# renjie-liang/HUAL

Measured on AMD Instinct MI355X. Metric: train clips/sec, higher is better.
Workload: dtype f32 (fp16x3 / bf16x3 split-operand MFMA, fp32 accumulate); 1 GPU; Charades-STA SeqPAN train step (fwd+bwd+clip+AdamWD, dropout 0.2), batch 64/GPU, T=128, vdim=1024, L=20, C=8, dim=128, 8 heads, 2 attention layers, random init; ONE batch resident in HBM, batch assembly (hual_assemble_batch) outside the timed region; global_batch=64, T=128, vdim=1024, L=20, parallelism=dp1, launch=hipGraph, video_dtype=f32

## Files before the change

hual_amd/csrc/dablock.h:

```cpp
#pragma once
#include "common.h"
#include "rowops.h"

namespace hual {

#define HUAL_LNPROJ_MAX 5
struct LnProjArgs {
  const float* x;
  const float* xa; int pre_site; float* x_out;
  uint8_t* pre_bits; uint8_t* y1_bits;
  const float* x2;
  const float* g1; const float* b1; float* y1;
  int drop_site1;
  const float* g2; const float* b2; float* y2;
  float* mean; float* rstd;
  int nproj;
  const float* wimg[HUAL_LNPROJ_MAX];
  const float* bias[HUAL_LNPROJ_MAX];
  float* out[HUAL_LNPROJ_MAX]; int ldo[HUAL_LNPROJ_MAX];
  int src[HUAL_LNPROJ_MAX];
  int accum[HUAL_LNPROJ_MAX];
  int act[HUAL_LNPROJ_MAX];
  int out_site[HUAL_LNPROJ_MAX];
  uint8_t* out_bits[HUAL_LNPROJ_MAX];
// ... 51 lines not shown
  const float* pre_x; const float* pre_mean; const float* pre_rstd; const float* pre_g; const float* pre_dy; const float* pre_add;
};
int ln_proj_bwd_rows(int R, int Nv = 0);
int ln_proj_bwd_blocks(int R, int Nv = 0);
int launch_ln_proj_bwd(const LnProjBwdArgs& a, const DropCfg& drop, hipStream_t s);

struct DaMidBwdArgs {
  const float* dz1;
  const float *gate, *val, *sg, *xg, *sv, *xv;
  const float* w[10];
  float *d_sc, *d_val, *d_ln1a, *d_g, *dz_sg, *dz_xg, *d_sv, *d_xv, *d_satt, *d_xatt;
  int R; int MT; int Nv;
};
int launch_da_mid_bwd(const DaMidBwdArgs& a, hipStream_t s);

}
```

hual_amd/csrc/dablock.hip:

```cpp
#include "dablock.h"
#include "tilecore.h"
#include "prof.h"

using namespace hual;

__device__ __forceinline__ float row16_max(float v) {
  v = fmaxf(v, dpp_xor_partner(v, 1));
  v = fmaxf(v, dpp_xor_partner(v, 2));
  v = fmaxf(v, dpp_xor_partner(v, 4));
  v = fmaxf(v, dpp_xor_partner(v, 8));
  return v;
}
__device__ __forceinline__ float4 sig4(float4 v) { return make_float4(sigmoidf_(v.x), sigmoidf_(v.y), sigmoidf_(v.z), sigmoidf_(v.w)); }

#include "lnproj_body.h"

template <int NT, bool PLAIN>
__global__ __launch_bounds__(CB_THREADS) void ln_proj_kernel(LnProjArgs a, DropCfg drop) {
  extern __shared__ __attribute__((aligned(16))) char lp_lds[];
  ln_proj_body<NT, false, PLAIN>(a, drop, lp_lds);
}
template <int NT>
__global__ __launch_bounds__(CB_THREADS) void ln_proj_pair_kernel(LnProjArgs a0, LnProjArgs a1, DropCfg drop) {
  extern __shared__ __attribute__((aligned(16))) char lp_lds[];
// ... 271 lines not shown
  }
}
template <int NT>
__global__ __launch_bounds__(CB_THREADS) void da_post_kernel(DaPostArgs a, DropCfg drop) {
  extern __shared__ __attribute__((aligned(16))) char dp_lds[];
  da_post_body<NT, false>(a, drop, nullptr, dp_lds);
}
template <int NT>
__global__ __launch_bounds__(CB_THREADS) void da_post_lnproj_kernel(DaPostArgs a, DropCfg drop, LnProjArgs lp) {
  extern __shared__ __attribute__((aligned(16))) char dp_lds[];
  da_post_body<NT, true>(a, drop, &lp, dp_lds);
}

#define LB_ROWS 48
#define LB_U (LB_ROWS / 16)
template <bool PRE, int NT, bool SIX = false>
__global__ __launch_bounds__(CB_THREADS) void ln_proj_bwd_kernel(LnProjBwdArgs a, DropCfg drop) {
  extern __shared__ __attribute__((aligned(16))) char lb_lds[];
  char* S0 = lb_lds;
  char* S1 = S0 + 2 * LB_ROWS * 256;
  char* Ps = S1 + 2 * LB_ROWS * 256;
  float* ainv0 = reinterpret_cast<float*>(Ps + 8 * 4 * 32 * 16);
  float* ainv1 = ainv0 + LB_ROWS;
  const int lane = threadIdx.x & 63, wave = threadIdx.x >> 6;
  const int l32 = threadIdx.x & 31, grp = threadIdx.x >> 5;
  const int col = 4 * l32;
  const int MT = a.MT, R = a.R;
  const int tile_ = xcd_tile_clip(blockIdx.x, R, a.Nv, MT);
  if (tile_ < 0) return;
  const int r0 = tile_ * MT;
  const int RE = min(R, r0 + MT);
  const int j = lane & 15, g = lane >> 4, ecol = 16 * wave + 4 * g;
  const DropRegs dr = drop_load(drop);

  TfW w[2];
  tf_load_w(w[0], a.wimg_t[0], wave, lane);
  float4 nv[LB_U], xv[LB_U], a1v[LB_U];
  float mu[LB_U], rsd[LB_U];
  constexpr bool pre = PRE;
  const float* add1p = pre ? (a.pre_add ? a.pre_add : a.x) : (a.add1 ? a.add1 : a.x);
  const float* a0p = pre ? a.pre_dy : a.A[0];
  const int lda0 = pre ? HUAL_D : a.lda[0];
  uint32_t nkb[LB_U];
  const int nsteps = SIX ? 6 : a.nsteps;
  auto has_bits = [&](int k) { return !SIX && a.a_bits[k] != nullptr; };
  auto to_second = [&](int k) { return SIX ? k >= 4 : a.dst[k] != 0; };
  const bool has_g2 = SIX || a.g2 != nullptr, has_add_dy1 = SIX || a.add_dy1 != nullptr, has_dy1_bits = !SIX && a.dy1_bits != nullptr;
  const uint8_t* kb0p = has_bits(0) ? a.a_bits[0] : reinterpret_cast<const uint8_t*>(a.x);
  float4 pxv[LB_U];
  float pmu[LB_U], prs[LB_U];
#pragma unroll
  for (int u = 0; u < LB_U; ++u) {
    const int row = min(r0 + grp + 16 * u, R - 1);
    nv[u] = ld4(a0p + (size_t)row * lda0 + col);
    nkb[u] = SIX ? 0u : kb0p[(size_t)row * 16 + (l32 >> 1)];
    xv[u] = ld4(a.x + (size_t)row * HUAL_D + col);
    a1v[u] = ld4(add1p + (size_t)row * HUAL_D + col);
    mu[u] = a.mean[row];
    rsd[u] = a.rstd[row];
    if (pre) { pxv[u] = ld4(a.pre_x + (size_t)row * HUAL_D + col); pmu[u] = a.pre_mean[row]; prs[u] = a.pre_rstd[row]; }
  }
  const float4 g1 = ld4(a.g1 + col);
  float4 sg2 = f4zero(), sb2 = f4zero();
  if (pre) {
    const float4 pg = ld4(a.pre_g + col);
#pragma unroll
    for (int u = 0; u < LB_U; ++u) {
      const int lr = grp + 16 * u;
      const bool ok = lr < MT && r0 + lr < RE;
      const float4 v = pxv[u], dy = nv[u];
      const float mean = pmu[u], rstd = prs[u];
      const float4 xh = make_float4((v.x - mean) * rstd, (v.y - mean) * rstd, (v.z - mean) * rstd, (v.w - mean) * rstd);
      if (ok) { sb2 = cb_add(sb2, dy); sg2 = cb_fma(dy, xh, sg2); }
      const float4 gv = cb_mul(dy, pg);
      const float m1 = fast_sum32(cb_hsum(gv)) * (1.0f / HUAL_D);
      const float m2 = fast_sum32(cb_hsum(cb_mul(gv, xh))) * (1.0f / HUAL_D);
      float4 dx = make_float4(rstd * (gv.x - m1 - xh.x * m2), rstd * (gv.y - m1 - xh.y * m2),
                              rstd * (gv.z - m1 - xh.z * m2), rstd * (gv.w - m1 - xh.w * m2));
      if (a.pre_add) dx = make_float4(__fadd_rn(dx.x, a1v[u].x), __fadd_rn(dx.y, a1v[u].y), __fadd_rn(dx.z, a1v[u].z), __fadd_rn(dx.w, a1v[u].w));
      nv[u] = dx;
      a1v[u] = dx;
    }
  }
  const float4 g2 = has_g2 ? ld4(a.g2 + col) : f4zero();
  float4 addt[NT];
  const float* addp = has_add_dy1 ? a.add_dy1 : a.x;
#pragma unroll
  for (int rt = 0; rt < NT; ++rt) addt[rt] = SIX ? f4zero() : ld4(addp + (uint32_t)min(r0 + 16 * rt + j, R - 1) * (uint32_t)HUAL_D + (uint32_t)ecol);
  auto fill = [&](int k) {
    char* S = (k & 1) ? S1 : S0;
    float* ai = (k & 1) ? ainv1 : ainv0;
#pragma unroll
    for (int u = 0; u < LB_U; ++u) {
      const int lr = grp + 16 * u, row = r0 + lr;
      if (lr >= MT) continue;
      const bool ok = row < RE;
      float4 v = ok ? nv[u] : f4zero();
      if (has_bits(k)) {
        if (dr.enabled) v = f4_select((nkb[u] >> (4 * (l32 & 1))) & 15u, make_float4(v.x * dr.scale, v.y * dr.scale, v.z * dr.scale, v.w * dr.scale));
        if (ok && a.a_save[k]) st4_nt(a.a_save[k] + (size_t)row * HUAL_D + col, v);
      }
      const float inv = cb_store_operand(S, S + LB_ROWS * 256, lr, l32, v);
      if (l32 == 0) ai[lr] = ok ? inv : 0.f;
// ... 1 lines not shown
  };
  HUAL_STAMP_K(4, 0);
  fill(0);
  HUAL_STAMP_K(4, 1);
  float4 acc0[NT], acc1[NT];
  bool first0 = true, first1 = true;
#pragma unroll
  for (int rt = 0; rt < NT; ++rt) { acc0[rt] = f4zero(); acc1[rt] = f4zero(); }
#pragma unroll
  for (int k = 0; k < HUAL_LNBWD_MAX; ++k) {
    if (k >= nsteps) break;
    const bool more = k + 1 < nsteps;
    if (SIX && k == 5) {
#pragma unroll
      for (int rt = 0; rt < NT; ++rt) addt[rt] = ld4(addp + (uint32_t)min(r0 + 16 * rt + j, R - 1) * (uint32_t)HUAL_D + (uint32_t)ecol);
    }
    if (more) {
      const uint8_t* nbp = has_bits(k + 1) ? a.a_bits[k + 1] : reinterpret_cast<const uint8_t*>(a.x);
      const float* nap = a.A[k + 1];
      const int nld = a.lda[k + 1];
#pragma unroll
      for (int u = 0; u < LB_U; ++u) {
        const size_t row = (size_t)min(r0 + grp + 16 * u, R - 1);
        nv[u] = ld4(nap + row * nld + col);
        nkb[u] = SIX ? 0u : nbp[row * 16 + (l32 >> 1)];
      }
      tf_load_w(w[(k + 1) & 1], a.wimg_t[k + 1], wave, lane);
    }
    cb_barrier();
    HUAL_STAMP_K(4, 2 + 3 * k);
// ... 28 lines not shown
    float4 v = acc0[rt];
    if (has_add_dy1) v = cb_add(v, addt[rt]);
    D0[lr * 32 + (ecol >> 2)] = v;
    if (has_g2) D1[lr * 32 + (ecol >> 2)] = acc1[rt];
  }
  uint32_t kb1[LB_U], kbz[LB_U];
  {
    const uint8_t* b1p = has_dy1_bits ? a.dy1_bits : reinterpret_cast<const uint8_t*>(a.x);
    const uint8_t* bzp = a.dz_bits ? a.dz_bits : reinterpret_cast<const uint8_t*>(a.x);
#pragma unroll
    for (int u = 0; u < LB_U; ++u) {
      const size_t row = (size_t)min(r0 + grp + 16 * u, R - 1);
      kb1[u] = SIX ? 0u : b1p[row * 16 + (l32 >> 1)];
      kbz[u] = bzp[row * 16 + (l32 >> 1)];
    }
  }
  cb_barrier();
  HUAL_STAMP_K(4, 21);
  float4 sg1 = f4zero(), sb1 = f4zero();
#pragma unroll
  for (int u = 0; u < LB_U; ++u) {
    const int lr = grp + 16 * u, row = r0 + lr;
    if (lr >= MT || row >= R) continue;
    const size_t off = (size_t)row * HUAL_D + col;
    const float4 v = xv[u];
    const float mean = mu[u], rstd = rsd[u];
    const float4 xh = make_float4((v.x - mean) * rstd, (v.y - mean) * rstd, (v.z - mean) * rstd, (v.w - mean) * rstd);
    float4 dy = D0[lr * 32 + l32];
    if (has_dy1_bits && dr.enabled) dy = f4_select((kb1[u] >> (4 * (l32 & 1))) & 15u, make_float4(dy.x * dr.scale, dy.y * dr.scale, dy.z * dr.scale, dy.w * dr.scale));
    sb1 = cb_add(sb1, dy);
    sg1 = cb_fma(dy, xh, sg1);
    float4 gv = cb_mul(dy, g1);
    if (has_g2) {
      const float4 dy2 = D1[lr * 32 + l32];
      sb2 = cb_add(sb2, dy2);
      sg2 = cb_fma(dy2, xh, sg2);
      gv = cb_fma(dy2, g2, gv);
    }
    const float m1 = fast_sum32(cb_hsum(gv)) * (1.0f / HUAL_D);
    const float m2 = fast_sum32(cb_hsum(cb_mul(gv, xh))) * (1.0f / HUAL_D);
    float4 dx = make_float4(rstd * (gv.x - m1 - xh.x * m2), rstd * (gv.y - m1 - xh.y * m2),
                            rstd * (gv.z - m1 - xh.z * m2), rstd * (gv.w - m1 - xh.w * m2));
    if (SIX || a.add1 || pre) dx = make_float4(__fadd_rn(dx.x, a1v[u].x), __fadd_rn(dx.y, a1v[u].y), __fadd_rn(dx.z, a1v[u].z), __fadd_rn(dx.w, a1v[u].w));
    st4(a.dx + off, dx);
    if (a.dz) {
      if (a.dz_bits && dr.enabled) dx = f4_select((kbz[u] >> (4 * (l32 & 1))) & 15u, make_float4(dx.x * dr.scale, dx.y * dr.scale, dx.z * dr.scale, dx.w * dr.scale));
      st4(a.dz + off, dx);
    }
  }
  HUAL_STAMP_K(4, 22);
  {
    auto xor32_sum = [&](float v) {
      const unsigned x = __builtin_bit_cast(unsigned, v);
      const auto r = __builtin_amdgcn_permlane32_swap(x, x, false, false);
      return v + __builtin_bit_cast(float, (lane & 32) ? r[0] : r[1]);
    };
    auto xor32_sum4 = [&](float4 v) { return make_float4(xor32_sum(v.x), xor32_sum(v.y), xor32_sum(v.z), xor32_sum(v.w)); };
    sg1 = xor32_sum4(sg1); sb1 = xor32_sum4(sb1); sg2 = xor32_sum4(sg2); sb2 = xor32_sum4(sb2);
    float4* pb = reinterpret_cast<float4*>(Ps);
    if (lane < 32) {
      float4* dst = pb + wave * 4 * 32 + l32;
      dst[0] = sg1; dst[32] = sb1; dst[64] = sg2; dst[96] = sb2;
    }
    cb_barrier();
    const float* pf = reinterpret_cast<const float*>(pb);
    const int e = threadIdx.x;
    float s = 0.f;
#pragma unroll
    for (int w = 0; w < 8; ++w) s += pf[w * 4 * HUAL_D + e];
    a.part[(size_t)tile_ * 4 * HUAL_D + e] = s;
  }
  HUAL_STAMP_K(4, 23);
}

template <int NT>
__global__ __launch_bounds__(CB_THREADS) void da_mid_bwd_kernel(DaMidBwdArgs a) {
  extern __shared__ __attribute__((aligned(16))) char dm_lds[];
  char* P0 = dm_lds;
  char* P1 = P0 + DP_SLOT;
  char* P2 = P1 + DP_SLOT;
  float* ainv0 = reinterpret_cast<float*>(P2 + DP_SLOT);
  float* ainv1 = ainv0 + DP_ROWS;
  float* ainv2 = ainv1 + DP_ROWS;
  float* smaxA = ainv2 + DP_ROWS;
  float* smaxB = smaxA + 8 * DP_ROWS;
  const int lane = threadIdx.x & 63, wave = threadIdx.x >> 6;
  const int l32 = threadIdx.x & 31, grp = threadIdx.x >> 5;
  const int col = 4 * l32;
  const int MT = a.MT, R = a.R;
  const int tile_ = xcd_tile_clip(blockIdx.x, R, a.Nv, MT);
  if (tile_ < 0) return;
  const int r0 = tile_ * MT;
  const int RE = min(R, r0 + MT);
  const int j = lane & 15, g = lane >> 4, ecol = 16 * wave + 4 * g;

  TfW wa, wb;
  tf_load_w(wa, a.w[0], wave, lane);
  {
    float4 zv[3];
#pragma unroll
    for (int u = 0; u < 3; ++u) zv[u] = ld4(a.dz1 + (size_t)min(r0 + grp + 16 * u, R - 1) * HUAL_D + col);
#pragma unroll
    for (int u = 0; u < 3; ++u) {
      const int lr = grp + 16 * u;
      if (lr >= MT) continue;
      const bool ok = r0 + lr < RE;
      const float inv = cb_store_operand(P1, P1 + DP_PLANE, lr, l32, ok ? zv[u] : f4zero());
      if (l32 == 0) ainv1[lr] = ok ? inv : 0.f;
    }
  }
  f32x4 accp[NT];
  auto fold = [&](float4 (&acc)[NT], const float* ai, bool first) {
#pragma unroll
    for (int rt = 0; rt < NT; ++rt) {
      const float ir = ai[16 * rt + j];
      if (first) acc[rt] = make_float4(fmaf(accp[rt][0], ir, 0.f), fmaf(accp[rt][1], ir, 0.f), fmaf(accp[rt][2], ir, 0.f), fmaf(accp[rt][3], ir, 0.f));
// ... 29 lines not shown
      const float sc = f16_row_scale(fmaxf(fmaxf(fmaxf(ma.x, ma.y), fmaxf(ma.z, ma.w)), fmaxf(fmaxf(mb.x, mb.y), fmaxf(mb.z, mb.w))), inv);
      uint2 h, l;
      f16_split4(f4scale1(v[rt], sc), h, l);
      const int off = tile256_off(lr, ecol >> 3) + 8 * (g & 1);
      *reinterpret_cast<uint2*>(P + off) = h;
      *reinterpret_cast<uint2*>(P + DP_PLANE + off) = l;
      if (wave == 0 && g == 0) ai[lr] = (r0 + lr < RE) ? inv : 0.f;
    }
  };
  auto zero_invalid = [&](float4 (&v)[NT]) {
#pragma unroll
    for (int rt = 0; rt < NT; ++rt) if (r0 + 16 * rt + j >= RE) v[rt] = f4zero();
  };

  float4 T1[NT], T2[NT], U1[NT], U2[NT], U3[NT], U4[NT];
  tf_load_w(wb, a.w[1], wave, lane);
  tile_ld(a.gate, U1);
  tile_ld(a.val, U2);
  cb_barrier();
  tf_mma_lean<NT, DP_PLANE>(P1, wa, lane, accp);
  tf_load_w(wa, a.w[2], wave, lane);
  fold(T1, ainv1, true);
#pragma unroll
  for (int rt = 0; rt < NT; ++rt) {
    const float4 d0 = T1[rt], gt = U1[rt], vl = U2[rt];
    T1[rt] = make_float4(d0.x * vl.x * gt.x * (1.f - gt.x), d0.y * vl.y * gt.y * (1.f - gt.y), d0.z * vl.z * gt.z * (1.f - gt.z),
                         d0.w * vl.w * gt.w * (1.f - gt.w));
    T2[rt] = cb_mul(d0, gt);
    save_nt(a.d_sc, rt, T1[rt]);
    save_nt(a.d_val, rt, T2[rt]);
  }
  zero_invalid(T1);
  zero_invalid(T2);
// ... 68 lines not shown
  zero_invalid(T2);
  put_max(smaxA, T1);
  put_max(smaxB, T2);
  cb_barrier();
  put_planes(P1, ainv1, smaxA, T1);
  put_planes(P0, ainv0, smaxB, T2);
  cb_barrier();
  tf_mma_lean<NT, DP_PLANE>(P1, wa, lane, accp);
  fold(T1, ainv1, true);
#pragma unroll
  for (int rt = 0; rt < NT; ++rt) save(a.d_satt, rt, T1[rt]);
  tf_mma_lean<NT, DP_PLANE>(P0, wb, lane, accp);
  fold(T2, ainv0, true);
#pragma unroll
  for (int rt = 0; rt < NT; ++rt) save(a.d_xatt, rt, T2[rt]);
}

#if defined(HUAL_STAMPS) && (HUAL_STAMPS == 1 || (HUAL_STAMPS >= 4 && HUAL_STAMPS <= 6))
extern "C" int hual_debug_stamps(unsigned long long* out, int n) {
  return (int)hipMemcpyFromSymbol(out, HIP_SYMBOL(g_hual_stamps), sizeof(unsigned long long) * (size_t)n);
}
extern "C" int hual_debug_stamps_reset() {
  static unsigned long long zeros[512 * HUAL_STAMP_SLOTS];
  return (int)hipMemcpyToSymbol(HIP_SYMBOL(g_hual_stamps), zeros, sizeof(zeros));
}
#endif

namespace hual {

static int tile_rows(int R, int Nv, int max_rows) { return xcd_clip_rows(R, Nv, 16, max_rows); }
// ... 110 lines not shown
  }
  HUAL_CHECK_HIP(hipGetLastError());
  return 0;
}

int ln_proj_bwd_rows(int R, int Nv) { return tile_rows(R, Nv, LB_ROWS); }
int ln_proj_bwd_blocks(int R, int Nv) { return cdiv(R, ln_proj_bwd_rows(R, Nv)); }

static bool ln_proj_bwd_six(const LnProjBwdArgs& a) {
  if (a.pre_x || a.nsteps != 6 || !a.g2 || !a.add_dy1 || a.dy1_bits || !a.add1) return false;
  for (int k = 0; k < 6; ++k)
    if (a.a_bits[k] || a.a_save[k] || (a.dst[k] != 0) != (k >= 4)) return false;
  return true;
}

int launch_ln_proj_bwd(const LnProjBwdArgs& a, const DropCfg& drop, hipStream_t s) {
  HUAL_REQUIRE(a.nsteps >= 1 && a.nsteps <= HUAL_LNBWD_MAX && a.R > 0, "ln_proj_bwd: step count / rows");
  HUAL_REQUIRE(a.MT >= 1 && a.MT <= LB_ROWS, "ln_proj_bwd: MT must be 1..48");
  HUAL_REQUIRE(a.x && a.mean && a.rstd && a.g1 && a.dx && a.part, "ln_proj_bwd: null tensor");
  bool any1 = false;
  for (int k = 0; k < a.nsteps; ++k) {
    HUAL_REQUIRE((a.A[k] || (k == 0 && a.pre_x)) && a.wimg_t[k] && (a.lda[k] % 4) == 0, "ln_proj_bwd: product operand");
    HUAL_REQUIRE(a.dst[k] == 0 || a.g2, "ln_proj_bwd: product for the absent second layer norm");
    any1 = any1 || a.dst[k] != 0;
  }
  HUAL_REQUIRE(!a.g2 || any1, "ln_proj_bwd: second layer norm without a product");
  HUAL_REQUIRE(!a.pre_x || (!a.g2 && !a.add1 && a.pre_mean && a.pre_rstd && a.pre_g && a.pre_dy), "ln_proj_bwd: layer-norm prologue");
  const size_t lds = (size_t)4 * LB_ROWS * 256 + 8 * 4 * 32 * 16 + 2 * LB_ROWS * sizeof(float);
  const double rows = (double)a.R;
  const double flops = 2.0 * rows * HUAL_D * HUAL_D * a.nsteps;
  const double bytes = 4.0 * (rows * HUAL_D * ((a.pre_x ? 7.0 : 4.0) + a.nsteps) + (double)a.nsteps * HUAL_D * HUAL_D);
  const dim3 grid(xcd_clip_grid(a.R, a.Nv, a.MT));
  const bool six = ln_proj_bwd_six(a);
#define LN_BWD_NT(NT)                                                                                                   \
  {                                                                                                                     \
    if (a.pre_x) { HUAL_DYN_LDS((ln_proj_bwd_kernel<true, NT>), 160 * 1024); HUAL_LAUNCH(flops, bytes, (ln_proj_bwd_kernel<true, NT>), grid, dim3(CB_THREADS), lds, s, a, drop); } \
    else if (six) { HUAL_DYN_LDS((ln_proj_bwd_kernel<false, NT, true>), 160 * 1024); HUAL_LAUNCH(flops, bytes, (ln_proj_bwd_kernel<false, NT, true>), grid, dim3(CB_THREADS), lds, s, a, drop); } \
    else { HUAL_DYN_LDS((ln_proj_bwd_kernel<false, NT>), 160 * 1024); HUAL_LAUNCH(flops, bytes, (ln_proj_bwd_kernel<false, NT>), grid, dim3(CB_THREADS), lds, s, a, drop); }      \
    break;                                                                                                              \
  }
  switch (cdiv(a.MT, 16)) {
    case 1: LN_BWD_NT(1)
    case 2: LN_BWD_NT(2)
    default: LN_BWD_NT(3)
  }
#undef LN_BWD_NT
  HUAL_CHECK_HIP(hipGetLastError());
  return 0;
}

int launch_da_mid_bwd(const DaMidBwdArgs& a, hipStream_t s) {
  HUAL_REQUIRE(a.dz1 && a.gate && a.val && a.sg && a.xg && a.sv && a.xv && a.R > 0, "da_mid_bwd: null / empty");
  HUAL_REQUIRE(a.MT >= 1 && a.MT <= DP_ROWS, "da_mid_bwd: MT must be 1..48");
  for (int k = 0; k < 10; ++k) HUAL_REQUIRE(a.w[k] != nullptr, "da_mid_bwd: null weight image");
  HUAL_REQUIRE(a.d_sc && a.d_val && a.d_ln1a && a.d_g && a.dz_sg && a.dz_xg && a.d_sv && a.d_xv && a.d_satt && a.d_xatt, "da_mid_bwd: null output");
  const size_t lds = (size_t)3 * DP_SLOT + (3 * DP_ROWS + 16 * DP_ROWS) * sizeof(float);
  const double rows = (double)a.R;
  const double flops = 10.0 * 2.0 * rows * HUAL_D * HUAL_D, bytes = 4.0 * (rows * HUAL_D * 17.0 + 10.0 * HUAL_D * HUAL_D);
  const dim3 grid(xcd_clip_grid(a.R, a.Nv, a.MT));
  switch (cdiv(a.MT, 16)) {
    case 1: { HUAL_DYN_LDS(da_mid_bwd_kernel<1>, 160 * 1024); HUAL_LAUNCH(flops, bytes, da_mid_bwd_kernel<1>, grid, dim3(CB_THREADS), lds, s, a); break; }
    case 2: { HUAL_DYN_LDS(da_mid_bwd_kernel<2>, 160 * 1024); HUAL_LAUNCH(flops, bytes, da_mid_bwd_kernel<2>, grid, dim3(CB_THREADS), lds, s, a); break; }
    default: { HUAL_DYN_LDS(da_mid_bwd_kernel<3>, 160 * 1024); HUAL_LAUNCH(flops, bytes, da_mid_bwd_kernel<3>, grid, dim3(CB_THREADS), lds, s, a); break; }
  }
  HUAL_CHECK_HIP(hipGetLastError());
  return 0;
}

}
```

hual_amd/csrc/prof.cpp:

```cpp
#include <stdlib.h>
#include "prof.h"
#include <map>
#include <string>
#include <vector>
#include <string.h>
#include "../../include/hual_seqpan.h"

namespace hual {

namespace {
struct Rec { std::string name; hipEvent_t a, b; double flops, bytes; };
struct Agg { std::string name; int64_t launches = 0; double usec = 0.0, flops = 0.0, bytes = 0.0; };
struct State {
  bool on = false;
  std::vector<Rec> recs;
  std::vector<Agg> aggs;
};
thread_local State g_prof;

std::string clean(const char* s) {
  std::string n(s);
  while (!n.empty() && (n.front() == '(' || n.front() == ' ')) n.erase(n.begin());
  while (!n.empty() && (n.back() == ')' || n.back() == ' ')) n.pop_back();
  return n;
// ... 56 lines not shown
  const Agg& a = g_prof.aggs[i];
  strncpy(name, a.name.c_str(), (size_t)name_cap - 1);
  name[name_cap - 1] = 0;
  if (launches) *launches = a.launches;
  if (usec) *usec = a.usec;
  if (flops) *flops = a.flops;
  if (bytes) *bytes = a.bytes;
  return 0;
}

int hual_prof_kernel_pipe(const char* kernel, int* pipe, int* passes) {
  if (!kernel || !pipe || !passes) return HUAL_ERR_INVALID;
  struct Row { const char* prefix; int pipe, passes; };
  static const Row rows[] = {
      {"conv_block_", HUAL_PIPE_MATRIX16, 3}, {"ln_proj", HUAL_PIPE_MATRIX16, 3}, {"da_post", HUAL_PIPE_MATRIX16, 3},
      {"da_mid_bwd", HUAL_PIPE_MATRIX16, 3},  {"mproj_", HUAL_PIPE_MATRIX16, 3},
      {"feature_", HUAL_PIPE_MATRIX16, 3},    {"dw_f16_", HUAL_PIPE_MATRIX16, 3},
      {"attn_", HUAL_PIPE_MATRIX16, 3},      {"cq_fwd_staged", HUAL_PIPE_MATRIX16, 3}, {"cq_bwd_staged", HUAL_PIPE_MATRIX16, 3},
      {"cq_", HUAL_PIPE_MATRIX32, 1},
  };
  for (const Row& r : rows)
    if (strncmp(kernel, r.prefix, strlen(r.prefix)) == 0) { *pipe = r.pipe; *passes = r.passes; return 0; }
  *pipe = HUAL_PIPE_NONE; *passes = 0;
  return 0;
}

}
```

hual_amd/csrc/seqpan.hip:

```cpp
#include "attn.h"
#include "prof.h"
#include "cq.h"
#include "convblock.h"
#include "dablock.h"
#include "embed.h"
#include "gemm.h"
#include "heads.h"
#include "mproj.h"
#include "optim.h"
#include "params.h"
#include "rowops.h"
#include <stdlib.h>
#include <string.h>
#include <algorithm>
#include <unordered_map>
#include <vector>

namespace hual {
const char* last_error_cstr();
}
using namespace hual;

namespace {

// ... 80 lines not shown
  }
  void ln_bwd_split(const LnBwd& a0, float* dg_lo, float* db_lo, float* dg_hi, float* db_hi, const PosBwdJob* pos = nullptr, int npos = 0) {
    LnBwd a = a0;
    const int nlo = ln_bwd_blocks(a.split), nhi = ln_bwd_blocks(a.R - a.split);
    a.part = buf("part." + std::to_string(part_seq++), (size_t)(nlo + nhi) * 4, HUAL_D);
    ColsumJob cj{};
    cj.src = a.part; cj.nblk = nlo; cj.nvec = 4;
    cj.dst[0] = dg_lo; cj.dst[1] = db_lo;
    if (active) colsum.push_back(cj);
    cj.src = a.part + (size_t)nlo * 4 * HUAL_D; cj.nblk = nhi;
    cj.dst[0] = dg_hi; cj.dst[1] = db_hi;
    if (active) colsum.push_back(cj);
    if (live()) chk(launch_ln_bwd(a, drop, stream, pos, npos, &rs));
  }
  void ln_proj_bwd(const LnProjBwdArgs& a0, float* dg1, float* db1, float* dg2, float* db2) {
    LnProjBwdArgs a = a0;
    a.MT = ln_proj_bwd_rows(a.R, a.Nv);
    const int nblk = ln_proj_bwd_blocks(a.R, a.Nv);
    a.part = buf("part." + std::to_string(part_seq++), (size_t)nblk * 4, HUAL_D);
    ColsumJob cj{};
    cj.src = a.part; cj.nblk = nblk; cj.nvec = 4;
    cj.dst[0] = dg1; cj.dst[1] = db1; cj.dst[2] = dg2; cj.dst[3] = db2;
    if (active) colsum.push_back(cj);
    if (live()) chk(launch_ln_proj_bwd(a, drop, stream));
  }
  void flush_colsum(const EmbedUnpack* unpack = nullptr) {
    for (size_t i = 0; i < colsum.size() && !dry && ok(); i += HUAL_COLSUM_MAX_JOBS) {
      const bool last = i + HUAL_COLSUM_MAX_JOBS >= colsum.size();
      chk(launch_colsum(colsum.data() + i, (int)std::min<size_t>(HUAL_COLSUM_MAX_JOBS, colsum.size() - i), stream, last ? unpack : nullptr));
    }
    if (colsum.empty() && unpack && !dry && ok()) chk(launch_colsum(nullptr, 0, stream, unpack));
    colsum.clear();
  }
  void attn_fwd(const AttnJob* j, int n) { if (live()) chk(launch_attn_fwd(j, n, drop, stream)); }
  void attn_bwd(const AttnJob* j, int n) {
    if (live()) chk(launch_attn_bwd(j, n, drop, stream));
  }
};

// ... 773 lines not shown
    cqg.w0[i] = c.g(pm.cq[i].w0); cqg.w1[i] = c.g(pm.cq[i].w1); cqg.wm[i] = c.g(pm.cq[i].wm);
  }
  const int tri_nv = tri_bwd_blocks_v(c.rs), tri_nq = tri_bwd_blocks_q(c.rs);
  float* tri_part = c.buf("part." + std::to_string(c.part_seq++), (size_t)(tri_nv + tri_nq) * 3, D);
  for (int side = 0; side < 2; ++side) {
    ColsumJob cj{};
    cj.src = tri_part + (side == 0 ? 0 : (size_t)tri_nv * 3 * D); cj.nblk = side == 0 ? tri_nv : tri_nq; cj.nvec = 3;
    cj.dst[0] = cqg.wm[side]; cj.dst[1] = cqg.w0[side]; cj.dst[2] = cqg.w1[1 - side];
    if (c.active) c.colsum.push_back(cj);
  }
  if (c.live()) {
    c.chk(launch_cq_bwd_impl(cq, cg, c.rs, dXa, dXb, c.stream));
    if (c.ok()) c.chk(launch_tri_bwd_impl(cq, cg, cqp, tri_part, c.rs, c.drop, dXa, dXb, c.stream));
  }
  float* dx = cg.dX;
  for (int li = c.cfg->attn_layer - 1; li >= 0; --li) {
    const DualAttnP& d = pm.da[li];
    const std::string t = "da" + std::to_string(li);
    const int site = HUAL_SITE_DA + 8 * li;
    c.stage(ST_DA, li);
    float* xin = li == 0 ? c.act("cb.x4") : c.act("da" + std::to_string(li - 1) + ".out");
    float* ln1 = c.act(t + ".ln1");
    float* lnt = c.act(t + ".lnt");
    float* mean = c.vec(t + ".mean");
    float* rstd = c.vec(t + ".rstd");
    float* qkv = c.buf(t + ".qkv", R, 3 * D);
    float* ktvt = c.buf(t + ".ktvt", R, 2 * D);
    float* s_att = c.act(t + ".s_att");
    float* x_att = c.act(t + ".x_att");
    float* sv = c.act(t + ".s");
// ... 32 lines not shown
      j.npieces = 2; j.A[1] = gd; j.lda[1] = D; j.kw[1] = D; j.dW[1] = c.g(k == 0 ? d.bl1_d2 : d.bl2_d2);
      c.push_dw(j);
    }
    c.push_dw(mkdw(o, D, D, d_g, D, R, c.g(d.guided.k), c.g(d.guided.b)));
    c.push_dw(mkdw(sv, D, D, dz_sg, D, R, c.g(d.s_gate.k), c.g(d.s_gate.b)));
    c.push_dw(mkdw(xv, D, D, dz_xg, D, R, c.g(d.x_gate.k), c.g(d.x_gate.b)));
    c.push_dw(mkdw(s_att, D, D, d_sv, D, R, c.g(d.s_dense.k), c.g(d.s_dense.b)));
    c.push_dw(mkdw(x_att, D, D, d_xv, D, R, c.g(d.x_dense.k), c.g(d.x_dense.b)));
    {
      LnProjBwdArgs lb{};
      lb.nsteps = 1; lb.lda[0] = D; lb.wimg_t[0] = imgt(d.dense2.k); lb.dst[0] = 0;
      if (dz2_ready) { lb.A[0] = dz2; }
      else { lb.A[0] = dx; lb.a_bits[0] = c.bits(t + ".kb4", R); lb.a_save[0] = dz2; }
      lb.dy1_bits = c.bits(t + ".kb3", R); lb.x = res; lb.mean = mean2; lb.rstd = rstd2; lb.g1 = c.p(d.ln2.g); lb.add1 = dx;
      lb.dx = d_res; lb.dz = dz1; lb.dz_bits = c.bits(t + ".kb2", R); lb.R = R; lb.Nv = Nv; lb.drop_row0 = 0;
      c.ln_proj_bwd(lb, c.g(d.ln2.g), c.g(d.ln2.b), nullptr, nullptr);
      DaMidBwdArgs mb{};
      mb.dz1 = dz1; mb.gate = gate; mb.val = val; mb.sg = sg; mb.xg = xg; mb.sv = sv; mb.xv = xv;
      const size_t wo[10] = {d.dense1.k, d.bl1_d1, d.bl2_d1, d.bl1_d2, d.bl2_d2, d.guided.k, d.s_gate.k, d.x_gate.k, d.s_dense.k, d.x_dense.k};
      for (int k = 0; k < 10; ++k) mb.w[k] = c.nimg(wo[k]);
      mb.d_sc = d_sc; mb.d_val = d_val; mb.d_ln1a = d_ln1a; mb.d_g = d_g; mb.dz_sg = dz_sg; mb.dz_xg = dz_xg; mb.d_sv = d_sv; mb.d_xv = d_xv;
      mb.d_satt = d_satt; mb.d_xatt = d_xatt; mb.R = R; mb.Nv = Nv; mb.MT = da_post_rows(R, Nv);
      if (c.live()) c.chk(launch_da_mid_bwd(mb, c.stream));
    }
    float* dq_self = c.act(dt + ".q_self");
    float* dq_cross = c.act(dt + ".q_cross");
    float* d_qkv = c.buf(dt + ".qkv", R, 3 * D);
    float* d_ktvt = c.buf(dt + ".ktvt", R, 2 * D);
    {
      AttnJob a[4];
      for (int k = 0; k < 4; ++k) {
        attn_job_init(a[k]);
        a[k].Q = qkv; a[k].ldq = 3 * D; a[k].B = B; a[k].qmask = rowmask; a[k].kmask = rowmask; a[k].lddo = D; a[k].lddq = D;
        a[k].O = (k & 1) ? x_att : s_att; a[k].ldo = D;
      }
      a[0].K = qkv + D; a[0].V = qkv + 2 * D; a[0].ldkv = 3 * D; a[0].Tq = T; a[0].Tk = T; a[0].qrow0 = 0; a[0].krow0 = 0;
      a[0].dO = d_satt; a[0].dQ = dq_self; a[0].dK = d_qkv + D; a[0].dV = d_qkv + 2 * D; a[0].lddkv = 3 * D; a[0].drop_site = site + 0;
      a[1].K = ktvt; a[1].V = ktvt + D; a[1].ldkv = 2 * D; a[1].Tq = T; a[1].Tk = L; a[1].qrow0 = 0; a[1].krow0 = Nv;
// ... 11 lines not shown
    c.push_dw(mkdw(ln1, D, D, d_qkv + 2 * D, 3 * D, R, c.g(d.f_value.k), c.g(d.f_value.b)));
    c.push_dw(mkdw(lnt, D, D, d_ktvt, 2 * D, R, c.g(d.t_key.k), c.g(d.t_key.b)));
    c.push_dw(mkdw(lnt, D, D, d_ktvt + D, 2 * D, R, c.g(d.t_value.k), c.g(d.t_value.b)));
    float* d_xin = c.act(dt + ".in");
    float* nz = nullptr; const uint8_t* nz_bits = nullptr;
    if (li > 0) { nz = c.act("d.da" + std::to_string(li - 1) + ".z2"); nz_bits = c.bits("da" + std::to_string(li - 1) + ".kb4", R); }
    {
      LnProjBwdArgs lb{};
      lb.nsteps = 6;
      const float* As[6] = {dq_self, dq_cross, d_qkv + D, d_qkv + 2 * D, d_ktvt, d_ktvt + D};
      const int lds_[6] = {D, D, 3 * D, 3 * D, 2 * D, 2 * D};
      const size_t wo[6] = {d.query.k, d.query.k, d.f_key.k, d.f_value.k, d.t_key.k, d.t_value.k};
      for (int k = 0; k < 6; ++k) { lb.A[k] = As[k]; lb.lda[k] = lds_[k]; lb.wimg_t[k] = imgt(wo[k]); lb.dst[k] = k < 4 ? 0 : 1; }
      lb.add_dy1 = d_ln1a; lb.x = xin; lb.mean = mean; lb.rstd = rstd; lb.g1 = c.p(d.ln1.g); lb.g2 = c.p(d.lnt.g);
      lb.add1 = d_res; lb.dx = d_xin; lb.dz = nz; lb.dz_bits = nz_bits; lb.R = R; lb.Nv = Nv; lb.drop_row0 = 0;
      c.ln_proj_bwd(lb, c.g(d.ln1.g), c.g(d.ln1.b), c.g(d.lnt.g), c.g(d.lnt.b));
    }
    dx = d_xin;
  }
  float* x0 = c.act("cb.x0");
  c.stage(ST_CONV);
  float* d_x0 = conv_block_bwd(c, "cb", x0, dx, pm.cb, c.rs, HUAL_SITE_CONV);
  c.stage(ST_ALWAYS);
  PosBwdJob pj[2];
  int npj = 0;
  if (!c.dry && c.stage_on(ST_INPUT)) pj[npj++] = PosBwdJob{{d_x0, nullptr}, c.g(pm.pos), 1, 1};
  if (!c.dry && c.stage_on(ST_PRED)) pj[npj++] = PosBwdJob{{fe_dx0[1], fe_dx0[0]}, c.g(pm.fe_pos), 1, 0};
  const bool pos_rides = c.sel_stage < 0;
  if (c.live() && npj && !pos_rides) c.chk(launch_pos_bwd(pj, npj, c.rs, c.stream));
  c.stage(ST_INPUT);
  float* lin = c.act("lin");
// ... 390 lines not shown
```

Before: 53100 clips/s.

## Fuse dual-attention backward stages into one chained per-tile kernel

Adds a kernel that runs, per row tile, the previous layer's six-product layer-norm backward, this layer's layer_norm_2 projection backward, and the middle dual-attention backward in sequence. Intermediate dx/dz tiles stay in registers instead of going through HBM. The next phase's weights and row data are prefetched while the current phase finishes. This cuts two kernel launches and several global round-trips per layer, at the cost of higher register pressure and a larger LDS footprint. It is on by default and can be disabled with an environment variable.

```diff
diff --git a/hual_amd/csrc/dablock.h b/hual_amd/csrc/dablock.h
--- a/hual_amd/csrc/dablock.h
+++ b/hual_amd/csrc/dablock.h
@@ -89,4 +89,6 @@
 };
 int launch_da_mid_bwd(const DaMidBwdArgs& a, hipStream_t s);
 
+int launch_da_top_mid_bwd(const LnProjBwdArgs* six, const LnProjBwdArgs& top, const DaMidBwdArgs& mid, const DropCfg& drop, hipStream_t s);
+
 }
diff --git a/hual_amd/csrc/dablock.hip b/hual_amd/csrc/dablock.hip
--- a/hual_amd/csrc/dablock.hip
+++ b/hual_amd/csrc/dablock.hip
@@ -309,9 +309,32 @@
 
 #define LB_ROWS 48
 #define LB_U (LB_ROWS / 16)
-template <bool PRE, int NT, bool SIX = false>
-__global__ __launch_bounds__(CB_THREADS) void ln_proj_bwd_kernel(LnProjBwdArgs a, DropCfg drop) {
-  extern __shared__ __attribute__((aligned(16))) char lb_lds[];
+#define LB_LDS (4 * LB_ROWS * 256 + 8 * 4 * 32 * 16 + 2 * LB_ROWS * 4)
+struct LbHand { float4 dx[LB_U], dz[LB_U]; };
+struct LbPre { TfW w0; float4 xv[LB_U]; float mu[LB_U], rsd[LB_U]; float4 g1; };
+#ifndef LB_HOIST
+#define LB_HOIST 2
+#endif
+#ifndef DM_HOIST
+#define DM_HOIST 3
+#endif
+__device__ __forceinline__ void lb_prefetch(const LnProjBwdArgs& a, int tile_, LbPre& p) {
+  const int lane = threadIdx.x & 63, wave = threadIdx.x >> 6;
+  const int l32 = threadIdx.x & 31, grp = threadIdx.x >> 5;
+  const int r0 = tile_ * a.MT;
+  if (LB_HOIST >= 1) tf_load_w(p.w0, a.wimg_t[0], wave, lane);
+  if (LB_HOIST < 2) return;
+#pragma unroll
+  for (int u = 0; u < LB_U; ++u) {
+    const int row = min(r0 + grp + 16 * u, a.R - 1);
+    p.xv[u] = ld4(a.x + (size_t)row * HUAL_D + 4 * l32);
+    p.mu[u] = a.mean[row];
+    p.rsd[u] = a.rstd[row];
+  }
+  p.g1 = ld4(a.g1 + 4 * l32);
+}
+template <bool PRE, int NT, bool SIX, bool IN, bool OUT, bool ONE, class Next>
+__device__ __forceinline__ void ln_proj_bwd_body(const LnProjBwdArgs& a, const DropCfg& drop, char* lb_lds, int tile_, LbHand& h, const LbPre& pre_in, Next&& next) {
   char* S0 = lb_lds;
   char* S1 = S0 + 2 * LB_ROWS * 256;
   char* Ps = S1 + 2 * LB_ROWS * 256;
@@ -321,15 +344,14 @@
   const int l32 = threadIdx.x & 31, grp = threadIdx.x >> 5;
   const int col = 4 * l32;
   const int MT = a.MT, R = a.R;
-  const int tile_ = xcd_tile_clip(blockIdx.x, R, a.Nv, MT);
-  if (tile_ < 0) return;
   const int r0 = tile_ * MT;
   const int RE = min(R, r0 + MT);
   const int j = lane & 15, g = lane >> 4, ecol = 16 * wave + 4 * g;
   const DropRegs dr = drop_load(drop);
 
   TfW w[2];
-  tf_load_w(w[0], a.wimg_t[0], wave, lane);
+  if (IN && LB_HOIST >= 1) w[0] = pre_in.w0;
+  else tf_load_w(w[0], a.wimg_t[0], wave, lane);
   float4 nv[LB_U], xv[LB_U], a1v[LB_U];
   float mu[LB_U], rsd[LB_U];
   constexpr bool pre = PRE;
@@ -337,9 +359,9 @@
   const float* a0p = pre ? a.pre_dy : a.A[0];
   const int lda0 = pre ? HUAL_D : a.lda[0];
   uint32_t nkb[LB_U];
-  const int nsteps = SIX ? 6 : a.nsteps;
-  auto has_bits = [&](int k) { return !SIX && a.a_bits[k] != nullptr; };
-  auto to_second = [&](int k) { return SIX ? k >= 4 : a.dst[k] != 0; };
+  const int nsteps = SIX ? 6 : (ONE ? 1 : a.nsteps);
+  auto has_bits = [&](int k) { return !SIX && !(IN && k == 0) && a.a_bits[k] != nullptr; };
+  auto to_second = [&](int k) { return SIX ? k >= 4 : (!ONE && a.dst[k] != 0); };
   const bool has_g2 = SIX || a.g2 != nullptr, has_add_dy1 = SIX || a.add_dy1 != nullptr, has_dy1_bits = !SIX && a.dy1_bits != nullptr;
   const uint8_t* kb0p = has_bits(0) ? a.a_bits[0] : reinterpret_cast<const uint8_t*>(a.x);
   float4 pxv[LB_U];
@@ -347,15 +369,21 @@
 #pragma unroll
   for (int u = 0; u < LB_U; ++u) {
     const int row = min(r0 + grp + 16 * u, R - 1);
+    if (IN) {
+      nv[u] = h.dz[u]; nkb[u] = 0u; a1v[u] = h.dx[u];
+      if (LB_HOIST >= 2) { xv[u] = pre_in.xv[u]; mu[u] = pre_in.mu[u]; rsd[u] = pre_in.rsd[u]; }
+      else { xv[u] = ld4(a.x + (size_t)row * HUAL_D + col); mu[u] = a.mean[row]; rsd[u] = a.rstd[row]; }
+      continue;
+    }
     nv[u] = ld4(a0p + (size_t)row * lda0 + col);
     nkb[u] = SIX ? 0u : kb0p[(size_t)row * 16 + (l32 >> 1)];
     xv[u] = ld4(a.x + (size_t)row * HUAL_D + col);
-    a1v[u] = ld4(add1p + (size_t)row * HUAL_D + col);
+    a1v[u] = (SIX && OUT) ? f4zero() : ld4(add1p + (size_t)row * HUAL_D + col);
     mu[u] = a.mean[row];
     rsd[u] = a.rstd[row];
     if (pre) { pxv[u] = ld4(a.pre_x + (size_t)row * HUAL_D + col); pmu[u] = a.pre_mean[row]; prs[u] = a.pre_rstd[row]; }
   }
-  const float4 g1 = ld4(a.g1 + col);
+  const float4 g1 = (IN && LB_HOIST >= 2) ? pre_in.g1 : ld4(a.g1 + col);
   float4 sg2 = f4zero(), sb2 = f4zero();
   if (pre) {
     const float4 pg = ld4(a.pre_g + col);
@@ -381,7 +409,7 @@
   float4 addt[NT];
   const float* addp = has_add_dy1 ? a.add_dy1 : a.x;
 #pragma unroll
-  for (int rt = 0; rt < NT; ++rt) addt[rt] = SIX ? f4zero() : ld4(addp + (uint32_t)min(r0 + 16 * rt + j, R - 1) * (uint32_t)HUAL_D + (uint32_t)ecol);
+  for (int rt = 0; rt < NT; ++rt) addt[rt] = (SIX || ONE) ? f4zero() : ld4(addp + (uint32_t)min(r0 + 16 * rt + j, R - 1) * (uint32_t)HUAL_D + (uint32_t)ecol);
   auto fill = [&](int k) {
     char* S = (k & 1) ? S1 : S0;
     float* ai = (k & 1) ? ainv1 : ainv0;
@@ -413,6 +441,10 @@
     if (SIX && k == 5) {
 #pragma unroll
       for (int rt = 0; rt < NT; ++rt) addt[rt] = ld4(addp + (uint32_t)min(r0 + 16 * rt + j, R - 1) * (uint32_t)HUAL_D + (uint32_t)ecol);
+      if (OUT) {
+#pragma unroll
+        for (int u = 0; u < LB_U; ++u) a1v[u] = ld4(add1p + (size_t)min(r0 + grp + 16 * u, R - 1) * HUAL_D + col);
+      }
     }
     if (more) {
       const uint8_t* nbp = has_bits(k + 1) ? a.a_bits[k + 1] : reinterpret_cast<const uint8_t*>(a.x);
@@ -471,6 +503,11 @@
       kb1[u] = SIX ? 0u : b1p[row * 16 + (l32 >> 1)];
       kbz[u] = bzp[row * 16 + (l32 >> 1)];
     }
+  }
+  next();
+  if (OUT) {
+#pragma unroll
+    for (int u = 0; u < LB_U; ++u) { h.dx[u] = f4zero(); h.dz[u] = f4zero(); }
   }
   cb_barrier();
   HUAL_STAMP_K(4, 21);
@@ -500,9 +537,11 @@
                             rstd * (gv.z - m1 - xh.z * m2), rstd * (gv.w - m1 - xh.w * m2));
     if (SIX || a.add1 || pre) dx = make_float4(__fadd_rn(dx.x, a1v[u].x), __fadd_rn(dx.y, a1v[u].y), __fadd_rn(dx.z, a1v[u].z), __fadd_rn(dx.w, a1v[u].w));
     st4(a.dx + off, dx);
-    if (a.dz) {
+    if (OUT) h.dx[u] = dx;
+    if (OUT || a.dz) {
       if (a.dz_bits && dr.enabled) dx = f4_select((kbz[u] >> (4 * (l32 & 1))) & 15u, make_float4(dx.x * dr.scale, dx.y * dr.scale, dx.z * dr.scale, dx.w * dr.scale));
-      st4(a.dz + off, dx);
+      if (OUT) { h.dz[u] = dx; if (a.dz) st4_nt(a.dz + off, dx); }
+      else st4(a.dz + off, dx);
     }
   }
   HUAL_STAMP_K(4, 22);
@@ -529,10 +568,34 @@
   }
   HUAL_STAMP_K(4, 23);
 }
-
+template <bool PRE, int NT, bool SIX = false>
+__global__ __launch_bounds__(CB_THREADS) void ln_proj_bwd_kernel(LnProjBwdArgs a, DropCfg drop) {
+  extern __shared__ __attribute__((aligned(16))) char lb_lds[];
+  const int tile_ = xcd_tile_clip(blockIdx.x, a.R, a.Nv, a.MT);
+  if (tile_ < 0) return;
+  LbHand h;
+  LbPre pre;
+  ln_proj_bwd_body<PRE, NT, SIX, false, false, false>(a, drop, lb_lds, tile_, h, pre, [] {});
+}
+
+#define DM_LDS (3 * DP_SLOT + (3 * DP_ROWS + 16 * DP_ROWS) * 4)
+template <int NT> struct DmPre { TfW wa, wb; float4 gate[NT], val[NT]; };
 template <int NT>
-__global__ __launch_bounds__(CB_THREADS) void da_mid_bwd_kernel(DaMidBwdArgs a) {
-  extern __shared__ __attribute__((aligned(16))) char dm_lds[];
+__device__ __forceinline__ void dm_prefetch(const DaMidBwdArgs& a, int tile_, DmPre<NT>& p) {
+  const int lane = threadIdx.x & 63, wave = threadIdx.x >> 6;
+  const int r0 = tile_ * a.MT;
+  if (DM_HOIST >= 1) tf_load_w(p.wa, a.w[0], wave, lane);
+  if (DM_HOIST >= 2) tf_load_w(p.wb, a.w[1], wave, lane);
+  if (DM_HOIST < 3) return;
+#pragma unroll
+  for (int rt = 0; rt < NT; ++rt) {
+    const uint32_t eo = (uint32_t)min(r0 + 16 * rt + (lane & 15), a.R - 1) * (uint32_t)HUAL_D + (uint32_t)(16 * wave + 4 * (lane >> 4));
+    p.gate[rt] = ld4(a.gate + eo);
+    p.val[rt] = ld4(a.val + eo);
+  }
+}
+template <int NT, bool IN>
+__device__ __forceinline__ void da_mid_bwd_body(const DaMidBwdArgs& a, char* dm_lds, int tile_, const float4 (&zin)[3], const DmPre<NT>& pre_in) {
   char* P0 = dm_lds;
   char* P1 = P0 + DP_SLOT;
   char* P2 = P1 + DP_SLOT;
@@ -545,18 +608,17 @@
   const int l32 = threadIdx.x & 31, grp = threadIdx.x >> 5;
   const int col = 4 * l32;
   const int MT = a.MT, R = a.R;
-  const int tile_ = xcd_tile_clip(blockIdx.x, R, a.Nv, MT);
-  if (tile_ < 0) return;
   const int r0 = tile_ * MT;
   const int RE = min(R, r0 + MT);
   const int j = lane & 15, g = lane >> 4, ecol = 16 * wave + 4 * g;
 
   TfW wa, wb;
-  tf_load_w(wa, a.w[0], wave, lane);
+  if (IN && DM_HOIST >= 1) wa = pre_in.wa;
+  else tf_load_w(wa, a.w[0], wave, lane);
   {
     float4 zv[3];
 #pragma unroll
-    for (int u = 0; u < 3; ++u) zv[u] = ld4(a.dz1 + (size_t)min(r0 + grp + 16 * u, R - 1) * HUAL_D + col);
+    for (int u = 0; u < 3; ++u) zv[u] = IN ? zin[u] : ld4(a.dz1 + (size_t)min(r0 + grp + 16 * u, R - 1) * HUAL_D + col);
 #pragma unroll
     for (int u = 0; u < 3; ++u) {
       const int lr = grp + 16 * u;
@@ -616,9 +678,15 @@
   };
 
   float4 T1[NT], T2[NT], U1[NT], U2[NT], U3[NT], U4[NT];
-  tf_load_w(wb, a.w[1], wave, lane);
-  tile_ld(a.gate, U1);
-  tile_ld(a.val, U2);
+  if (IN && DM_HOIST >= 2) wb = pre_in.wb;
+  else tf_load_w(wb, a.w[1], wave, lane);
+  if (IN && DM_HOIST >= 3) {
+#pragma unroll
+    for (int rt = 0; rt < NT; ++rt) { U1[rt] = pre_in.gate[rt]; U2[rt] = pre_in.val[rt]; }
+  } else {
+    tile_ld(a.gate, U1);
+    tile_ld(a.val, U2);
+  }
   cb_barrier();
   tf_mma_lean<NT, DP_PLANE>(P1, wa, lane, accp);
   tf_load_w(wa, a.w[2], wave, lane);
@@ -717,6 +785,37 @@
   fold(T2, ainv0, true);
 #pragma unroll
   for (int rt = 0; rt < NT; ++rt) save(a.d_xatt, rt, T2[rt]);
+}
+template <int NT>
+__global__ __launch_bounds__(CB_THREADS) void da_mid_bwd_kernel(DaMidBwdArgs a) {
+  extern __shared__ __attribute__((aligned(16))) char dm_lds[];
+  const int tile_ = xcd_tile_clip(blockIdx.x, a.R, a.Nv, a.MT);
+  if (tile_ < 0) return;
+  const float4 zin[3] = {};
+  DmPre<NT> pre;
+  da_mid_bwd_body<NT, false>(a, dm_lds, tile_, zin, pre);
+}
+
+struct DaChainArgs { LnProjBwdArgs six, top; DaMidBwdArgs mid; DropCfg drop; };
+template <int NT, bool SIXF>
+__global__ __launch_bounds__(CB_THREADS) void da_top_mid_bwd_kernel(DaChainArgs) {
+  extern __shared__ __attribute__((aligned(16))) char dc_lds[];
+  const DaChainArgs& ka = *(const DaChainArgs*)(const __attribute__((address_space(4))) DaChainArgs*)__builtin_amdgcn_kernarg_segment_ptr();
+  const LnProjBwdArgs& six = ka.six;
+  const LnProjBwdArgs& top = ka.top;
+  const DaMidBwdArgs& mid = ka.mid;
+  const DropCfg& drop = ka.drop;
+  const int tile_ = xcd_tile_clip(blockIdx.x, top.R, top.Nv, top.MT);
+  if (tile_ < 0) return;
+  LbHand h;
+  LbPre tp;
+  DmPre<NT> mp;
+  auto own = [](int t) { asm volatile("" : "+s"(t)); return t; };
+  const int t_top = own(tile_), t_mid = own(tile_);
+  if (SIXF) ln_proj_bwd_body<false, NT, true, false, true, false>(six, drop, dc_lds, tile_, h, tp, [&] { lb_prefetch(top, t_top, tp); });
+  ln_proj_bwd_body<false, NT, false, SIXF, true, true>(top, drop, dc_lds, t_top, h, tp, [&] { dm_prefetch<NT>(mid, t_mid, mp); });
+  cb_barrier();
+  da_mid_bwd_body<NT, true>(mid, dc_lds, t_mid, h.dz, mp);
 }
 
 #if defined(HUAL_STAMPS) && (HUAL_STAMPS == 1 || (HUAL_STAMPS >= 4 && HUAL_STAMPS <= 6))
@@ -857,7 +956,7 @@
   return true;
 }
 
-int launch_ln_proj_bwd(const LnProjBwdArgs& a, const DropCfg& drop, hipStream_t s) {
+static int check_ln_proj_bwd(const LnProjBwdArgs& a) {
   HUAL_REQUIRE(a.nsteps >= 1 && a.nsteps <= HUAL_LNBWD_MAX && a.R > 0, "ln_proj_bwd: step count / rows");
   HUAL_REQUIRE(a.MT >= 1 && a.MT <= LB_ROWS, "ln_proj_bwd: MT must be 1..48");
   HUAL_REQUIRE(a.x && a.mean && a.rstd && a.g1 && a.dx && a.part, "ln_proj_bwd: null tensor");
@@ -869,10 +968,20 @@
   }
   HUAL_REQUIRE(!a.g2 || any1, "ln_proj_bwd: second layer norm without a product");
   HUAL_REQUIRE(!a.pre_x || (!a.g2 && !a.add1 && a.pre_mean && a.pre_rstd && a.pre_g && a.pre_dy), "ln_proj_bwd: layer-norm prologue");
-  const size_t lds = (size_t)4 * LB_ROWS * 256 + 8 * 4 * 32 * 16 + 2 * LB_ROWS * sizeof(float);
+  return 0;
+}
+static void ln_proj_bwd_work(const LnProjBwdArgs& a, double& flops, double& bytes) {
   const double rows = (double)a.R;
-  const double flops = 2.0 * rows * HUAL_D * HUAL_D * a.nsteps;
-  const double bytes = 4.0 * (rows * HUAL_D * ((a.pre_x ? 7.0 : 4.0) + a.nsteps) + (double)a.nsteps * HUAL_D * HUAL_D);
+  flops += 2.0 * rows * HUAL_D * HUAL_D * a.nsteps;
+  bytes += 4.0 * (rows * HUAL_D * ((a.pre_x ? 7.0 : 4.0) + a.nsteps) + (double)a.nsteps * HUAL_D * HUAL_D);
+}
+
+int launch_ln_proj_bwd(const LnProjBwdArgs& a, const DropCfg& drop, hipStream_t s) {
+  int rc = check_ln_proj_bwd(a);
+  if (rc) return rc;
+  const size_t lds = LB_LDS;
+  double flops = 0.0, bytes = 0.0;
+  ln_proj_bwd_work(a, flops, bytes);
   const dim3 grid(xcd_clip_grid(a.R, a.Nv, a.MT));
   const bool six = ln_proj_bwd_six(a);
 #define LN_BWD_NT(NT)                                                                                                   \
@@ -892,12 +1001,18 @@
   return 0;
 }
 
-int launch_da_mid_bwd(const DaMidBwdArgs& a, hipStream_t s) {
+static int check_da_mid_bwd(const DaMidBwdArgs& a) {
   HUAL_REQUIRE(a.dz1 && a.gate && a.val && a.sg && a.xg && a.sv && a.xv && a.R > 0, "da_mid_bwd: null / empty");
   HUAL_REQUIRE(a.MT >= 1 && a.MT <= DP_ROWS, "da_mid_bwd: MT must be 1..48");
   for (int k = 0; k < 10; ++k) HUAL_REQUIRE(a.w[k] != nullptr, "da_mid_bwd: null weight image");
   HUAL_REQUIRE(a.d_sc && a.d_val && a.d_ln1a && a.d_g && a.dz_sg && a.dz_xg && a.d_sv && a.d_xv && a.d_satt && a.d_xatt, "da_mid_bwd: null output");
-  const size_t lds = (size_t)3 * DP_SLOT + (3 * DP_ROWS + 16 * DP_ROWS) * sizeof(float);
+  return 0;
+}
+
+int launch_da_mid_bwd(const DaMidBwdArgs& a, hipStream_t s) {
+  int rc = check_da_mid_bwd(a);
+  if (rc) return rc;
+  const size_t lds = DM_LDS;
   const double rows = (double)a.R;
   const double flops = 10.0 * 2.0 * rows * HUAL_D * HUAL_D, bytes = 4.0 * (rows * HUAL_D * 17.0 + 10.0 * HUAL_D * HUAL_D);
   const dim3 grid(xcd_clip_grid(a.R, a.Nv, a.MT));
@@ -910,4 +1025,41 @@
   return 0;
 }
 
-}
+int launch_da_top_mid_bwd(const LnProjBwdArgs* six, const LnProjBwdArgs& top, const DaMidBwdArgs& mid, const DropCfg& drop, hipStream_t s) {
+  int rc = check_ln_proj_bwd(top);
+  if (rc) return rc;
+  if ((rc = check_da_mid_bwd(mid))) return rc;
+  HUAL_REQUIRE(top.nsteps == 1 && top.dst[0] == 0 && !top.pre_x && !top.g2 && !top.add_dy1 && top.add1 && top.dz == mid.dz1, "da_top_mid_bwd: the layer_norm_2 phase must feed the middle");
+  HUAL_REQUIRE(top.R == mid.R && top.Nv == mid.Nv && top.MT == mid.MT, "da_top_mid_bwd: the phases must share rows and tiles");
+  static_assert(LB_ROWS == DP_ROWS, "the phases share the tile height");
+  const size_t lds = LB_LDS > DM_LDS ? LB_LDS : DM_LDS;
+  const double rows = (double)top.R;
+  double flops = 10.0 * 2.0 * rows * HUAL_D * HUAL_D, bytes = 4.0 * (rows * HUAL_D * 16.0 + 10.0 * HUAL_D * HUAL_D);
+  ln_proj_bwd_work(top, flops, bytes);
+  if (six) {
+    if ((rc = check_ln_proj_bwd(*six))) return rc;
+    HUAL_REQUIRE(ln_proj_bwd_six(*six) && six->dz && six->dz == top.A[0] && six->dx == top.add1 && !top.a_bits[0],
+                 "da_top_mid_bwd: the six-product phase must feed the layer_norm_2 phase");
+    HUAL_REQUIRE(six->R == top.R && six->Nv == top.Nv && six->MT == top.MT, "da_top_mid_bwd: the phases must share rows and tiles");
+    ln_proj_bwd_work(*six, flops, bytes);
+    bytes -= 4.0 * rows * HUAL_D * 2.0;
+  }
+  const dim3 grid(xcd_clip_grid(top.R, top.Nv, top.MT));
+  const DaChainArgs ka{six ? *six : top, top, mid, drop};
+#define DA_CHAIN_NT(NT)                                                                                                                        \
+  {                                                                                                                                            \
+    if (six) { HUAL_DYN_LDS((da_top_mid_bwd_kernel<NT, true>), 160 * 1024); HUAL_LAUNCH(flops, bytes, (da_top_mid_bwd_kernel<NT, true>), grid, dim3(CB_THREADS), lds, s, ka); } \
+    else { HUAL_DYN_LDS((da_top_mid_bwd_kernel<NT, false>), 160 * 1024); HUAL_LAUNCH(flops, bytes, (da_top_mid_bwd_kernel<NT, false>), grid, dim3(CB_THREADS), lds, s, ka); } \
+    break;                                                                                                                                     \
+  }
+  switch (cdiv(top.MT, 16)) {
+    case 1: DA_CHAIN_NT(1)
+    case 2: DA_CHAIN_NT(2)
+    default: DA_CHAIN_NT(3)
+  }
+#undef DA_CHAIN_NT
+  HUAL_CHECK_HIP(hipGetLastError());
+  return 0;
+}
+
+}
diff --git a/hual_amd/csrc/prof.cpp b/hual_amd/csrc/prof.cpp
--- a/hual_amd/csrc/prof.cpp
+++ b/hual_amd/csrc/prof.cpp
@@ -94,7 +94,7 @@
   struct Row { const char* prefix; int pipe, passes; };
   static const Row rows[] = {
       {"conv_block_", HUAL_PIPE_MATRIX16, 3}, {"ln_proj", HUAL_PIPE_MATRIX16, 3}, {"da_post", HUAL_PIPE_MATRIX16, 3},
-      {"da_mid_bwd", HUAL_PIPE_MATRIX16, 3},  {"mproj_", HUAL_PIPE_MATRIX16, 3},
+      {"da_mid_bwd", HUAL_PIPE_MATRIX16, 3},  {"da_top_mid_bwd", HUAL_PIPE_MATRIX16, 3}, {"mproj_", HUAL_PIPE_MATRIX16, 3},
       {"feature_", HUAL_PIPE_MATRIX16, 3},    {"dw_f16_", HUAL_PIPE_MATRIX16, 3},
       {"attn_", HUAL_PIPE_MATRIX16, 3},      {"cq_fwd_staged", HUAL_PIPE_MATRIX16, 3}, {"cq_bwd_staged", HUAL_PIPE_MATRIX16, 3},
       {"cq_", HUAL_PIPE_MATRIX32, 1},
diff --git a/hual_amd/csrc/seqpan.hip b/hual_amd/csrc/seqpan.hip
--- a/hual_amd/csrc/seqpan.hip
+++ b/hual_amd/csrc/seqpan.hip
@@ -118,6 +118,10 @@
     if (live()) chk(launch_ln_bwd(a, drop, stream, pos, npos, &rs));
   }
   void ln_proj_bwd(const LnProjBwdArgs& a0, float* dg1, float* db1, float* dg2, float* db2) {
+    const LnProjBwdArgs a = ln_proj_bwd_prep(a0, dg1, db1, dg2, db2);
+    if (live()) chk(launch_ln_proj_bwd(a, drop, stream));
+  }
+  LnProjBwdArgs ln_proj_bwd_prep(const LnProjBwdArgs& a0, float* dg1, float* db1, float* dg2, float* db2) {
     LnProjBwdArgs a = a0;
     a.MT = ln_proj_bwd_rows(a.R, a.Nv);
     const int nblk = ln_proj_bwd_blocks(a.R, a.Nv);
@@ -126,7 +130,7 @@
     cj.src = a.part; cj.nblk = nblk; cj.nvec = 4;
     cj.dst[0] = dg1; cj.dst[1] = db1; cj.dst[2] = dg2; cj.dst[3] = db2;
     if (active) colsum.push_back(cj);
-    if (live()) chk(launch_ln_proj_bwd(a, drop, stream));
+    return a;
   }
   void flush_colsum(const EmbedUnpack* unpack = nullptr) {
     for (size_t i = 0; i < colsum.size() && !dry && ok(); i += HUAL_COLSUM_MAX_JOBS) {
@@ -930,6 +934,10 @@
     if (c.ok()) c.chk(launch_tri_bwd_impl(cq, cg, cqp, tri_part, c.rs, c.drop, dXa, dXb, c.stream));
   }
   float* dx = cg.dX;
+  static const bool da_bwd_split = getenv("HUAL_DA_BWD_SPLIT") != nullptr && atoi(getenv("HUAL_DA_BWD_SPLIT")) != 0;
+  const bool da_bwd_fused = !da_bwd_split && c.sel_stage < 0;
+  LnProjBwdArgs six_pend{};
+  bool have_six = false;
   for (int li = c.cfg->attn_layer - 1; li >= 0; --li) {
     const DualAttnP& d = pm.da[li];
     const std::string t = "da" + std::to_string(li);
@@ -992,14 +1000,16 @@
       else { lb.A[0] = dx; lb.a_bits[0] = c.bits(t + ".kb4", R); lb.a_save[0] = dz2; }
       lb.dy1_bits = c.bits(t + ".kb3", R); lb.x = res; lb.mean = mean2; lb.rstd = rstd2; lb.g1 = c.p(d.ln2.g); lb.add1 = dx;
       lb.dx = d_res; lb.dz = dz1; lb.dz_bits = c.bits(t + ".kb2", R); lb.R = R; lb.Nv = Nv; lb.drop_row0 = 0;
-      c.ln_proj_bwd(lb, c.g(d.ln2.g), c.g(d.ln2.b), nullptr, nullptr);
+      const LnProjBwdArgs top = c.ln_proj_bwd_prep(lb, c.g(d.ln2.g), c.g(d.ln2.b), nullptr, nullptr);
+      if (!da_bwd_fused && c.live()) c.chk(launch_ln_proj_bwd(top, c.drop, c.stream));
       DaMidBwdArgs mb{};
       mb.dz1 = dz1; mb.gate = gate; mb.val = val; mb.sg = sg; mb.xg = xg; mb.sv = sv; mb.xv = xv;
       const size_t wo[10] = {d.dense1.k, d.bl1_d1, d.bl2_d1, d.bl1_d2, d.bl2_d2, d.guided.k, d.s_gate.k, d.x_gate.k, d.s_dense.k, d.x_dense.k};
       for (int k = 0; k < 10; ++k) mb.w[k] = c.nimg(wo[k]);
       mb.d_sc = d_sc; mb.d_val = d_val; mb.d_ln1a = d_ln1a; mb.d_g = d_g; mb.dz_sg = dz_sg; mb.dz_xg = dz_xg; mb.d_sv = d_sv; mb.d_xv = d_xv;
       mb.d_satt = d_satt; mb.d_xatt = d_xatt; mb.R = R; mb.Nv = Nv; mb.MT = da_post_rows(R, Nv);
-      if (c.live()) c.chk(launch_da_mid_bwd(mb, c.stream));
+      if (c.live()) c.chk(da_bwd_fused ? launch_da_top_mid_bwd(have_six ? &six_pend : nullptr, top, mb, c.drop, c.stream) : launch_da_mid_bwd(mb, c.stream));
+      have_six = false;
     }
     float* dq_self = c.act(dt + ".q_self");
     float* dq_cross = c.act(dt + ".q_cross");
@@ -1041,7 +1051,12 @@
       for (int k = 0; k < 6; ++k) { lb.A[k] = As[k]; lb.lda[k] = lds_[k]; lb.wimg_t[k] = imgt(wo[k]); lb.dst[k] = k < 4 ? 0 : 1; }
       lb.add_dy1 = d_ln1a; lb.x = xin; lb.mean = mean; lb.rstd = rstd; lb.g1 = c.p(d.ln1.g); lb.g2 = c.p(d.lnt.g);
       lb.add1 = d_res; lb.dx = d_xin; lb.dz = nz; lb.dz_bits = nz_bits; lb.R = R; lb.Nv = Nv; lb.drop_row0 = 0;
-      c.ln_proj_bwd(lb, c.g(d.ln1.g), c.g(d.ln1.b), c.g(d.lnt.g), c.g(d.lnt.b));
+      if (da_bwd_fused && li > 0) {
+        six_pend = c.ln_proj_bwd_prep(lb, c.g(d.ln1.g), c.g(d.ln1.b), c.g(d.lnt.g), c.g(d.lnt.b));
+        have_six = true;
+      } else {
+        c.ln_proj_bwd(lb, c.g(d.ln1.g), c.g(d.ln1.b), c.g(d.lnt.g), c.g(d.lnt.b));
+      }
     }
     dx = d_xin;
   }
```

After: 53710 clips/s, median of 6. 1.2% higher.
